# jhwang7628/openpbso

Hardware: AMD Instinct MI355X
Metric: audio samples/s & real-time x at N_obj x N_modes (higher is better)
Workload: dtype f32

## Files before the change

openpbso_amd/csrc/kernels_block.hip:

```cpp
#include <type_traits>

#include "kernels.h"
#include "wave_ops.h"

namespace pbso {
namespace iir_block {

typedef float f4 __attribute__((ext_vector_type(4)));

constexpr int BJ = BLOCK_J, BN = BLOCK_N;
constexpr int GROUP = BJ * BN;
constexpr int ST_ROW = 130;
constexpr int ST_PAIR = 260;
__host__ __device__ constexpr int park_off(int n) { return (n & 7) * ST_PAIR + (n >> 3) * 32; }
constexpr int LIT_ROW = 68;
constexpr int ST_FLOATS = BLOCK_STAGE_FLOATS;
constexpr int RING = BLOCK_RING_FLOATS;
constexpr int FTM_U_ROW = 36;
constexpr int H_ROW = 72;
constexpr int H_PLANE = BN * H_ROW;
static_assert(BN * ST_ROW <= ST_FLOATS && 8 * ST_PAIR <= BN * ST_ROW && BJ * LIT_ROW <= ST_FLOATS && 2 * H_PLANE <= ST_FLOATS, "staging area");

struct BlkDims {
    int nb, m_pad, b_pad, frames, n_groups;
// ... 79 lines not shown
    float *__restrict__ b_qn = p_qnorm + ((size_t)obj * p.qn_nb + p.qn_b0) * p.m_pad + team.col0;
    constexpr bool HALF = R == 1;
    constexpr int RINGF = HALF ? BLOCK_HALF_RING_FLOATS : RING;
    constexpr int WAVE_FLOATS = ST_FLOATS + 2 * RINGF;
    float *stage = lds + wave * WAVE_FLOATS;
    float *ring = stage + ST_FLOATS;

    f2 x2[R], c1[R], c2[R];
    float t[R];
    bool dead[R];
#pragma unroll
    for (int r = 0; r < R; ++r) {
        const unsigned k = r * rowlen + utid;
        if (chunked) {
            const float *__restrict__ xsrc = p_xs + 2 * (((size_t)obj * p.n_chunks + chunk) * p.m_pad + team.col0);
            x2[r] = reinterpret_cast<const f2 *>(xsrc)[k];
        } else {
            x2[r].x = (p_sq + ubase)[k];
            x2[r].y = (p_sd + ubase)[k];
        }
        c1[r].x = (p_pc + ubase)[k];
        c2[r].x = (p_pc + p.plane + ubase)[k];
        c1[r].y = (p_pc + 2 * p.plane + ubase)[k];
        c2[r].y = (p_pc + 3 * p.plane + ubase)[k];
        dead[r] = b_ca[k] == 0.f && b_cb[k] == 0.f;
    }
    f4 wreg4[PROJ == 0 ? R : 1][8];
    u4 wq[PROJ == 1 ? R : 1][8];
#pragma unroll
    for (int r = 0; r < R; ++r) {
        const float *__restrict__ wsrc = p_wtab + ((ubase + r * rowlen + 64 * wave) / 2) * 64;
        if constexpr (PROJ == 0) {
#pragma unroll
            for (int i = 0; i < 8; ++i)
#pragma unroll
                for (int jj = 0; jj < 4; ++jj) wreg4[r][i][jj] = wsrc[(8 * (lane >> 4) + i) * 64 + 16 * jj + (lane & 15)];
        } else {
            const unsigned *__restrict__ wu = reinterpret_cast<const unsigned *>(wsrc);
#pragma unroll
            for (int i = 0; i < 8; ++i)
                wq[r][i] = u4{wu[(4 * i + 0) * 64 + lane], wu[(4 * i + 1) * 64 + lane], wu[(4 * i + 2) * 64 + lane], wu[(4 * i + 3) * 64 + lane]};
        }
    }

    constexpr bool FT = FORCED && PROJ == 0 && !QN && R <= 2;
    constexpr bool FTM = FT && R == 1;
    constexpr int U_ROW = FTM_U_ROW;
    float fB[FTM ? 4 : 1][2][4];
    if constexpr (FTM) {
#pragma unroll
        for (int tl = 0; tl < 4; ++tl)
#pragma unroll
            for (int c = 0; c < 2; ++c)
#pragma unroll
                for (int ks = 0; ks < 4; ++ks)
                    fB[tl][c][ks] = (p_ftab + (size_t)(2 * (4 * ks + (lane >> 4)) + c) * p.plane + ubase)[64 * wave + 16 * tl + (lane & 15)];
    }
    float fq[FT && !FTM ? R : 1][BJ], fd[FT && !FTM ? R : 1][BJ];
    if constexpr (FT && !FTM) {
#pragma unroll
        for (int r = 0; r < R; ++r) {
#pragma unroll
            for (int i = 0; i < BJ; ++i) {
                fq[r][i] = (p_ftab + (size_t)(2 * i) * p.plane + ubase)[r * rowlen + utid];
                fd[r][i] = (p_ftab + (size_t)(2 * i + 1) * p.plane + ubase)[r * rowlen + utid];
            }
        }
    }

    constexpr bool TAPS_VALU = FORCED && PROJ == 0 && R == 1;
    float phi[TAPS_VALU ? 16 : 1];
    if constexpr (TAPS_VALU) {
        const double ea = (double)b_ca[utid], eb = (double)b_cb[utid];
        double vq = 1.0, vd = 1.0;
        phi[0] = 1.f;
#pragma unroll
        for (int d = 1; d < 16; ++d) {
            vd = ea * vd + eb * vq;
            vq = vq + vd;
            phi[d] = dead[0] ? 0.f : (float)vq;
        }
    }

    bool scaled = false;
    auto usable = [](float x) { return x >= 0x1p-20f && x <= 0x1p40f; };
    auto rescale = [&](const float (&from)[R], const float (&tn)[R]) {
        bool ok = true, same = true, unit = true;
#pragma unroll
        for (int r = 0; r < R; ++r) {
            ok = ok && usable(tn[r]);
            same = same && tn[r] == from[r];
            unit = unit && from[r] == 1.f;
        }
        ok = __all(ok);
        if (ok) {
            if (!__all(same)) {
#pragma unroll
                for (int r = 0; r < R; ++r) {
                    const float f = tn[r] / from[r];
                    x2[r].x = x2[r].x * f;
                    x2[r].y = x2[r].y * f;
                }
            }
        } else if (!__all(unit)) {
#pragma unroll
            for (int r = 0; r < R; ++r) {
                x2[r].x = x2[r].x / from[r];
                x2[r].y = x2[r].y / from[r];
            }
        }
        scaled = ok;
    };
    {
        const int row0 = chunked ? p_xtrow[(size_t)obj * p.n_chunks + chunk] : p_xfer_init[obj];
        float s0[R];
#pragma unroll
        for (int r = 0; r < R; ++r) {
            s0[r] = chunked ? 1.f : (p_ss + ubase)[r * rowlen + utid];
            const float tr = row0 >= 0 ? (float)(p_xfer_rows + (size_t)row0 * p.m_pad + team.col0)[r * rowlen + utid] : 1e7f;
            t[r] = dead[r] ? 1.f : tr;
        }
        rescale(s0, t);
    }

    const BufDesc *__restrict__ dsc = p_desc + (size_t)obj * p.nb;
    float *__restrict__ aout = team.part_row >= 0 ? p_audio_parts + (size_t)team.part_row * p.audio_stride
                                                  : p_audio + (size_t)obj * p.audio_stride;
    const int B = p.frames;

    const f4 *bsrc = reinterpret_cast<const f4 *>(stage + park_off(lane & 15) + (lane >> 4) * 64);
    f2 *wdst = reinterpret_cast<f2 *>(stage + (lane >> 4) * 64 + 2 * (lane & 15));
    auto park = [&](int n, f2 v) { wdst[park_off(n) / 2] = v; };
    const f4 *lsrc = reinterpret_cast<const f4 *>(stage + (lane & 15) * LIT_ROW + (lane >> 4) * 16);

    auto wave_sync = [&]() {
        __builtin_amdgcn_fence(__ATOMIC_RELEASE, "wavefront");
        __builtin_amdgcn_wave_barrier();
        __builtin_amdgcn_fence(__ATOMIC_ACQUIRE, "wavefront");
    };


    float nca[R], ncb[R], ng11[R], ng12[R], ng22[R], ngr[R];
    const float *__restrict__ g32_obj = p_g32 + (size_t)p_g32_off[obj] * p.m_pad + team.col0;
    float *gland = lds + blockDim.x / 64 * WAVE_FLOATS + wave * (3 * R * 64);
    float ntr[R];
    auto lane_off = [&]() {
        unsigned v = utid;
        asm volatile("" : "+v"(v));
        return v;
    };
    const unsigned rowlen4 = 4u * rowlen;
    auto lane_off4 = [&]() { return 4u * lane_off(); };
    auto ld_row = [](const float *base, unsigned off) { return *reinterpret_cast<const float *>(reinterpret_cast<const char *>(base) + off); };
    auto st_row = [](float *base, unsigned off, float v) { *reinterpret_cast<float *>(reinterpret_cast<char *>(base) + off) = v; };
    const int dump_row = DUMP ? p_dump_row[obj] : -1;
    int dump_b = 0;
    auto dump_state = [&](int r, int blk) {
        if (DUMP && dump_row >= 0) {
            f2 *dst = reinterpret_cast<f2 *>(p_xdump) + (((size_t)dump_row * p.qn_nb + dump_b) * 32 + blk) * p.m_pad + team.col0;
            dst[r * rowlen + lane_off()] = x2[r];
        }
    };
    auto dump_scale = [&](int code) {
        if (DUMP && dump_row >= 0) {
            float *dst = p_xscale + ((size_t)dump_row * p.qn_nb + dump_b) * p.m_pad + team.col0;
            const unsigned off = lane_off4();
#pragma unroll
            for (int r = 0; r < R; ++r) st_row(dst, off + r * rowlen4, code > 0 ? t[r] : (float)code);
        }
    };
    auto prefetch_gq = [&]() {
        if (QN) {
            const unsigned off = lane_off4();
#pragma unroll
            for (int r = 0; r < R; ++r) {
                ng11[r] = ld_row(b_gq, off + r * rowlen4);
                ng12[r] = ld_row(b_gq + p.plane, off + r * rowlen4);
                ng22[r] = ld_row(b_gq + 2 * p.plane, off + r * rowlen4);
            }
        }
    };
    auto prefetch = [&](const BufDesc &nd, bool with_gq = true) {
        const unsigned off = lane_off4();
#pragma unroll
        for (int r = 0; r < R; ++r) {
            nca[r] = ld_row(b_ca, off + r * rowlen4);
            ncb[r] = ld_row(b_cb, off + r * rowlen4);
        }
        if (with_gq) prefetch_gq();
        if (nd.frow >= 0 && !(nd.flags & DESC_DIRECT)) {
            const float *__restrict__ gsrc = p_grows + (size_t)nd.frow * p.m_pad + team.col0;
#pragma unroll
            for (int r = 0; r < R; ++r) ngr[r] = ld_row(gsrc, off + r * rowlen4);
        }
        if (nd.trow >= 0) {
            const double *__restrict__ tsrc = p_xfer_rows + (size_t)nd.trow * p.m_pad + team.col0;
#pragma unroll
            for (int r = 0; r < R; ++r)
                ntr[r] = (float)*reinterpret_cast<const double *>(reinterpret_cast<const char *>(tsrc) + 2u * (off + r * rowlen4));
        }
    };

    const unsigned gland_addr = (unsigned)(size_t)gland;
    auto prefetch_direct = [&](const BufDesc &nd) {
        if (nd.frow >= 0 && (nd.flags & DESC_DIRECT)) {
            const unsigned voff = 4u * lane_off();
#pragma unroll
            for (int k = 0; k < 3; ++k) {
#pragma unroll
                for (int r = 0; r < R; ++r) {
                    const float *__restrict__ row = g32_obj + (size_t)(nd.frow + k) * p.m_pad + r * rowlen;
                    asm volatile("s_mov_b32 m0, %0\n\tglobal_load_lds_dword %1, %2"
                                 :: "s"(gland_addr + (unsigned)((k * R + r) * 256)), "v"(voff), "s"(row) : "memory", "m0");
                }
            }
        }
    };

    const unsigned park_base = (unsigned)(size_t)wdst;
    unsigned park_row[4];
#pragma unroll
    for (int j = 0; j < 4; ++j) park_row[j] = park_base + j * 2 * ST_PAIR * 4;
    auto step_p = [&](int r) {
        float qa, da, qn, dn;
        asm volatile("v_fma_f32 %0, %1, %2, %2" : "=v"(qa) : "v"(c1[r].x), "v"(x2[r].x));
        asm volatile("v_mul_f32 %0, %1, %2" : "=v"(da) : "v"(c1[r].y), "v"(x2[r].x));
        asm volatile("v_fma_f32 %0, %1, %2, %3" : "=v"(qn) : "v"(c2[r].x), "v"(x2[r].y), "v"(qa));
        asm volatile("v_fma_f32 %0, %1, %2, %3" : "=v"(dn) : "v"(c2[r].y), "v"(x2[r].y), "v"(da));
        x2[r].x = qn;
        x2[r].y = dn;
    };
#define PBSO_PK_PAIR(J, O0, O1)                                                                   \
    "v_pk_fma_f32 %[t], %[c1], %[x], %[x] op_sel_hi:[1,0,1]\n\t"                                   \
    "v_pk_fma_f32 %[y], %[c2], %[x], %[t] op_sel:[0,1,0] op_sel_hi:[1,1,1]\n\t"                    \
    "ds_write2_b64 %[a" #J "], %[x], %[y] offset0:" #O0 " offset1:" #O1 "\n\t"                      \
    "v_pk_fma_f32 %[t], %[c1], %[y], %[y] op_sel_hi:[1,0,1]\n\t"                                   \
    "v_pk_fma_f32 %[x], %[c2], %[y], %[t] op_sel:[0,1,0] op_sel_hi:[1,1,1]\n\t"
    static_assert(ST_PAIR / 2 == 130, "offsets of the ds_write2_b64 pairs below (8-byte units): blocks n, n + 1 are rows 130 apart, n + 8 is 16 further");
    auto vburst_pk = [&](int r) {
        f2 t, y;
        const f2 c2m = f2{c2[r].x, c2[r].y - 1.f};
        asm volatile(PBSO_PK_PAIR(0, 0, 130) PBSO_PK_PAIR(1, 0, 130) PBSO_PK_PAIR(2, 0, 130) PBSO_PK_PAIR(3, 0, 130)
                     PBSO_PK_PAIR(0, 16, 146) PBSO_PK_PAIR(1, 16, 146) PBSO_PK_PAIR(2, 16, 146) PBSO_PK_PAIR(3, 16, 146)
                     : [x] "+v"(x2[r]), [t] "=&v"(t), [y] "=&v"(y)
                     : [c1] "v"(c1[r]), [c2] "v"(c2m), [a0] "v"(park_row[0]), [a1] "v"(park_row[1]), [a2] "v"(park_row[2]), [a3] "v"(park_row[3])
                     : "memory");
    };
#undef PBSO_PK_PAIR
    auto coarse2 = [&](int r, auto nc, int blk) {
        constexpr int n = decltype(nc)::value;
        static_assert((n & 1) == 0 && park_off(n + 1) - park_off(n) == ST_PAIR, "a pair of blocks = two rows of the image");
        dump_state(r, blk);
        const f2 xa = x2[r];
        step_p(r);
        dump_state(r, blk + 1);
        asm volatile("ds_write2_b64 %0, %1, %2 offset0:%3 offset1:%4"
                     :: "v"(park_row[(n & 7) / 2]), "v"(xa), "v"(x2[r]), "n"((n >> 3) * 16), "n"((n >> 3) * 16 + ST_PAIR / 2) : "memory");
        step_p(r);
    };

    unsigned long long cy_head = 0, cy_pipe = 0, cy_bar = 0, cy_comb = 0, cy_mark = 0, cy_taps = 0, cy_step = 0;
    auto lap = [&](unsigned long long &acc) {
        if (p_census) {
            const unsigned long long now = __builtin_amdgcn_s_memtime();
            acc += now - cy_mark;
            cy_mark = now;
        }
    };
    BufDesc next = dsc[b_begin];
    prefetch(next);
    prefetch_direct(next);
    if (p_census) cy_mark = __builtin_amdgcn_s_memtime();
    int prio_rank = 0;
    if (p.rotate) {
        unsigned *word = p_board + 2048 + (((__builtin_amdgcn_s_getreg((31 << 11) | 20) & 7u) << 8) | ((__builtin_amdgcn_s_getreg((31 << 11) | 4) >> 8) & 0xFFu));
        if (tid == 0) ring[0] = __builtin_bit_cast(float, atomicAdd(word, 1u));
        __syncthreads();
        prio_rank = (int)(__builtin_bit_cast(unsigned, lds[ST_FLOATS]) & 3u);
        __syncthreads();
    }
    for (int b = b_begin; b < b_end; ++b) {
        const BufDesc cur = next;
        next = dsc[b + 1 < p.nb ? b + 1 : b];
        auto set_pipe_prio = [&]() {
            if (p.rotate) {
                switch ((prio_rank + b - b_begin) & 3) {
                case 0: __builtin_amdgcn_s_setprio(0); break;
                case 1: __builtin_amdgcn_s_setprio(1); break;
                case 2: __builtin_amdgcn_s_setprio(2); break;
                default: __builtin_amdgcn_s_setprio(3); break;
                }
            }
        };
        set_pipe_prio();

        const int frow = cur.frow;
        const int prow = (cur.flags & DESC_DIRECT) ? -1 : cur.prow;
        const float amp = cur.amp;
        const int trow = cur.trow;
        const uint32_t flags = cur.flags;
        float *rg = ring + (b & 1) * RING;
        auto ring_grp = [&](int grp) { return HALF ? ring + grp * RINGF : rg + GROUP * grp; };
        auto ring_s0 = [&]() { return HALF ? ring + GROUP : rg + GROUP * NG; };
        auto combine_half = [&](int grp) {
            if constexpr (HALF) {
                lap(cy_pipe);
                __syncthreads();
                lap(cy_bar);
                if (wave == (2 * (b - b_begin) + grp) % W) {
                    const float *r0 = lds + ST_FLOATS + grp * RINGF;
                    float *__restrict__ ao = aout + (size_t)b * B + GROUP * grp;
                    const unsigned j = lane_off() & 63u;
                    f4 acc = *reinterpret_cast<const f4 *>(r0 + 4 * j);
                    for (int w = 1; w < W; ++w) acc += *reinterpret_cast<const f4 *>(r0 + w * WAVE_FLOATS + 4 * j);
                    AUDIO_STORE(&ao[4 * j + 1], acc.x);
                    AUDIO_STORE(&ao[4 * j + 2], acc.y);
                    AUDIO_STORE(&ao[4 * j + 3], acc.z);
                    AUDIO_STORE(&ao[4 * j + 4], acc.w);
                    if (grp == 0 && j == 0) {
                        float a0 = r0[GROUP];
                        for (int w = 1; w < W; ++w) a0 += r0[w * WAVE_FLOATS + GROUP];
                        AUDIO_STORE(&ao[0], a0);
                    }
                }
                lap(cy_comb);
            }
        };
        dump_b = p.qn_b0 + b;

        if (flags & DESC_SKIP) {
            dump_scale(-1);
            const unsigned off = lane_off4();
            for (unsigned o = off; o < 4u * (unsigned)B; o += rowlen4) st_row(aout + (size_t)b * B, o, 0.f);
            if (QN) {
#pragma unroll
                for (int r = 0; r < R; ++r) st_row(b_qn + (size_t)b * p.m_pad, off + r * rowlen4, 0.f);
            }
            prefetch(next);
            prefetch_direct(next);
            continue;
        }
        if (trow != XFER_KEEP) {
            float tn[R], from[R];
#pragma unroll
            for (int r = 0; r < R; ++r) {
                const float tr = trow >= 0 ? ntr[r] : 1e7f;
                tn[r] = dead[r] ? 1.f : tr;
                from[r] = scaled ? t[r] : 1.f;
            }
            rescale(from, tn);
#pragma unroll
            for (int v = 0; v < R; ++v) t[v] = tn[v];
        }
        float g_[R];
#pragma unroll
        for (int r = 0; r < R; ++r) {
            float gv = ngr[r];
            if (flags & DESC_DIRECT) {
                __builtin_amdgcn_s_waitcnt(0x0F70);
                const float *gl = gland + r * 64 + lane;
                gv = __builtin_bit_cast(float, cur.prow) * gl[0];
                gv = fmaf(__builtin_bit_cast(float, cur.tile_mask), gl[R * 64], gv);
                gv = fmaf(__builtin_bit_cast(float, cur.pad[0]), gl[2 * R * 64], gv);
            }
            g_[r] = frow >= 0 ? (scaled ? gv * t[r] : gv) : 0.f;
        }
        prefetch_direct(next);
        const bool impulse = (flags & DESC_IMPULSE) != 0;
        const bool dense = frow >= 0 && !impulse;

        dump_scale(scaled && !dense ? 1 : 0);
        const bool forced_block = FORCED && PROJ == 0 && scaled && dense;
        if (scaled && !dense) {
            const bool hit0 = frow >= 0 && ((flags & DESC_DIRECT) || (cur.tile_mask & 1u));
            float p0 = 0.f;
#pragma unroll
            for (int v = 0; v < R; ++v) {
                float a = nca[v] * x2[v].y;
                a = fmaf(ncb[v], x2[v].x, a);
                if (hit0) a = fmaf(g_[v], amp, a);
                x2[v].y = a;
                x2[v].x = x2[v].x + a;
                p0 = (v == 0) ? x2[v].x : p0 + x2[v].x;
            }
            if (QN) {
                const unsigned off = lane_off4();
#pragma unroll
                for (int v = 0; v < R; ++v) {
                    float e = ng22[v] * x2[v].y * x2[v].y;
                    e = fmaf(ng12[v] * x2[v].x, x2[v].y, e);
                    e = fmaf(ng11[v] * x2[v].x, x2[v].x, e);
                    const float nrm = __builtin_amdgcn_sqrtf(fmaxf(e, 0.f));
                    st_row(b_qn + (size_t)b * p.m_pad, off + v * rowlen4, nrm * __builtin_amdgcn_rcpf(t[v]));
                }
            }
            p0 = wave_sum(p0);
            if (lane == 0) *ring_s0() = p0;

            if constexpr (PROJ == 0) {
            f4 bq[8];
            lap(cy_head);
            wave_sync();
            if constexpr (!DUMP) vburst_pk(0);
            else static_for<0, BN / 2>([&](auto hc) { coarse2(0, std::integral_constant<int, 2 * decltype(hc)::value>{}, 2 * decltype(hc)::value); });
            wave_sync();
#pragma unroll
            for (int i = 0; i < 8; ++i) bq[i] = bsrc[i];
            f4 acc0, acc1;
            static_for<0, U>([&](auto uc) {
                constexpr int u = decltype(uc)::value;
                constexpr int r = u % R, grp = u / R;
                constexpr int rn = (u + 1) % R;
                constexpr bool more = u + 1 < U;
                if constexpr (r == 0) {
                    acc0 = f4{0.f, 0.f, 0.f, 0.f};
                    acc1 = f4{0.f, 0.f, 0.f, 0.f};
                }
                wave_sync();
                __builtin_amdgcn_sched_barrier(0);
                if constexpr (more) {
                    if constexpr (!DUMP) vburst_pk(rn);
                    else static_for<0, BN / 2>([&](auto hc) {
                        constexpr int n = 2 * decltype(hc)::value;
                        coarse2(rn, std::integral_constant<int, n>{}, BN * ((u + 1) / R) + n);
                    });
                    wave_sync();
                }
                __builtin_amdgcn_sched_barrier(0);
                static_for<0, 32>([&](auto sc) {
                    constexpr int s = decltype(sc)::value;
                    if constexpr (s & 1) acc1 = __builtin_amdgcn_mfma_f32_16x16x4f32(wreg4[r][s >> 2][s & 3], bq[s >> 2][s & 3], acc1, 0, 0, 0);
                    else acc0 = __builtin_amdgcn_mfma_f32_16x16x4f32(wreg4[r][s >> 2][s & 3], bq[s >> 2][s & 3], acc0, 0, 0, 0);
                    if constexpr (more && (s & 3) == 3 && s >= 7) bq[(s >> 2) - 1] = bsrc[(s >> 2) - 1];
                    if constexpr (!more && s == 15) prefetch(next, false);
                    __builtin_amdgcn_sched_barrier(0);
                });
                if constexpr (more) bq[7] = bsrc[7];
                else prefetch_gq();
                if constexpr (r == R - 1) {
                    const f4 acc = acc0 + acc1;
                    const unsigned l = lane_off() & 63u;
                    *reinterpret_cast<f4 *>(ring_grp(grp) + 16 * (l & 15u) + 4 * (l >> 4)) = acc;
                    combine_half(grp);
                }
            });
            } else {
                unsigned *hdst = reinterpret_cast<unsigned *>(stage) + lane;
                const u4 *hsrc = reinterpret_cast<const u4 *>(reinterpret_cast<const unsigned *>(stage) + (lane & 15) * H_ROW + 4 * (lane >> 4));
                auto coarse16 = [&](int r, int n, int blk) {
                    dump_state(r, blk);
                    const f2 x = x2[r];
                    const float xq = x.x, xd = x.y;
                    const unsigned hq = __builtin_bit_cast(unsigned, xq) & 0xFFFF0000u;
                    const unsigned hd = __builtin_bit_cast(unsigned, xd) & 0xFFFF0000u;
                    const unsigned hp = __builtin_amdgcn_perm(hd, hq, 0x07060302u);
                    const float lq = xq - __builtin_bit_cast(float, hq), ld = xd - __builtin_bit_cast(float, hd);
                    const unsigned lp = __builtin_amdgcn_perm(__builtin_bit_cast(unsigned, ld), __builtin_bit_cast(unsigned, lq), 0x07060302u);
                    hdst[n * H_ROW] = hp;
                    hdst[H_PLANE + n * H_ROW] = lp;
                    const float qa = fmaf(c1[r].x, x.x, x.x);
                    const float da = c1[r].y * x.x;
                    x2[r].x = fmaf(c2[r].x, x.y, qa);
                    x2[r].y = fmaf(c2[r].y, x.y, da);
                };
                u4 breg[8];
                lap(cy_head);
                wave_sync();
#pragma unroll
                for (int n = 0; n < BN; ++n) coarse16(0, n, n);
                wave_sync();
#pragma unroll
                for (int g = 0; g < 4; ++g) {
                    breg[2 * g] = hsrc[4 * g];
                    breg[2 * g + 1] = hsrc[H_PLANE / 4 + 4 * g];
                }
                f4 acc0, acc1;
                static_for<0, U>([&](auto uc) {
                    constexpr int u = decltype(uc)::value;
                    constexpr int r = u % R, grp = u / R;
                    constexpr int rn = (u + 1) % R;
                    constexpr bool more = u + 1 < U;
                    if constexpr (r == 0) {
                        acc0 = f4{0.f, 0.f, 0.f, 0.f};
                        acc1 = f4{0.f, 0.f, 0.f, 0.f};
                    }
                    wave_sync();
                    __builtin_amdgcn_sched_barrier(0);
                    static_for<0, BN>([&](auto nc) {
                        constexpr int n = decltype(nc)::value;
                        if constexpr (more) coarse16(rn, n, BN * ((u + 1) / R) + n);
                        if constexpr (n >= 4) {
                            constexpr int k = n - 4, g = k / 3, which = k % 3;
                            const u4 wh = wq[r][2 * g], wl = wq[r][2 * g + 1];
                            if constexpr (which == 0)
                                acc0 = __builtin_amdgcn_mfma_f32_16x16x32_bf16(__builtin_bit_cast(bf16x8, wh), __builtin_bit_cast(bf16x8, breg[2 * g]), acc0, 0, 0, 0);
                            else if constexpr (which == 1)
                                acc1 = __builtin_amdgcn_mfma_f32_16x16x32_bf16(__builtin_bit_cast(bf16x8, wh), __builtin_bit_cast(bf16x8, breg[2 * g + 1]), acc1, 0, 0, 0);
                            else
                                acc0 = __builtin_amdgcn_mfma_f32_16x16x32_bf16(__builtin_bit_cast(bf16x8, wl), __builtin_bit_cast(bf16x8, breg[2 * g]), acc0, 0, 0, 0);
                        }
                        __builtin_amdgcn_sched_barrier(0);
                    });
                    if constexpr (more) {
                        wave_sync();
#pragma unroll
                        for (int g = 0; g < 4; ++g) {
                            breg[2 * g] = hsrc[4 * g];
                            breg[2 * g + 1] = hsrc[H_PLANE / 4 + 4 * g];
                        }
                    } else {
                        prefetch(next);
                    }
                    if constexpr (r == R - 1) {
                        const f4 acc = acc0 + acc1;
                        const unsigned l = lane_off() & 63u;
                        *reinterpret_cast<f4 *>(ring_grp(grp) + 16 * (l & 15u) + 4 * (l >> 4)) = acc;
                        combine_half(grp);
                    }
                });
            }
        } else if (forced_block) {
            if constexpr (PROJ == 0 && FORCED) {
            const float *__restrict__ tprow = p_tprof + (size_t)(prow >= 0 ? prow : 0) * p.b_pad;
            float *taps = stage + BN * ST_ROW;
            float qn[R];
            lap(cy_head);
            constexpr bool FIR_EARLY = R <= 2;
            float fir_ball[FIR_EARLY ? NG : 1][4];
            if constexpr (FIR_EARLY) {
#pragma unroll
                for (int grp = 0; grp < NG; ++grp)
#pragma unroll
                    for (int kk = 0; kk < 4; ++kk) fir_ball[grp][kk] = tprow[1 + GROUP * grp + BJ * (lane & 15) + 4 * kk + (lane >> 4)];
            }
            {
                const float tk0 = tprow[0];
                float p0 = 0.f, gs = 0.f;
#pragma unroll
                for (int v = 0; v < R; ++v) {
                    float a = nca[v] * x2[v].y;
                    a = fmaf(ncb[v], x2[v].x, a);
                    a = fmaf(g_[v], tk0, a);
                    x2[v].y = a;
                    x2[v].x = x2[v].x + a;
                    p0 = (v == 0) ? x2[v].x : p0 + x2[v].x;
                    gs = (v == 0) ? g_[v] : gs + g_[v];
                    qn[v] = x2[v].x * x2[v].x;
                }
                p0 = wave_sum(p0);
                if (!TAPS_VALU) gs = wave_sum(gs);
                if (lane == 0) *ring_s0() = p0;
                wave_sync();
                if (!TAPS_VALU && lane == 0) taps[0] = gs;
            }
            f4 bq[8];
            if constexpr (TAPS_VALU) {
                float pv[16];
#pragma unroll
                for (int d = 0; d < 16; ++d) pv[d] = g_[0] * phi[d];
                const float hd = wave_sum16(pv, lane, stage + ST_ROW, wave_sync);
                if (lane < 16) taps[taps_index(lane)] = hd;
                wave_sync();
            } else {
                f4 ah0 = f4{0.f, 0.f, 0.f, 0.f}, ah1 = f4{0.f, 0.f, 0.f, 0.f};
                static_for<0, R>([&](auto rc) {
                    constexpr int r = decltype(rc)::value;
                    if constexpr (r > 0) wave_sync();
                    park(0, f2{g_[r], g_[r]});
                    wave_sync();
#pragma unroll
                    for (int i = 0; i < 8; ++i) bq[i] = bsrc[i];
                    static_for<0, 32>([&](auto sc) {
                        constexpr int s2 = decltype(sc)::value;
                        if constexpr (s2 & 1) ah1 = __builtin_amdgcn_mfma_f32_16x16x4f32(wreg4[r][s2 >> 2][s2 & 3], bq[s2 >> 2][s2 & 3], ah1, 0, 0, 0);
                        else ah0 = __builtin_amdgcn_mfma_f32_16x16x4f32(wreg4[r][s2 >> 2][s2 & 3], bq[s2 >> 2][s2 & 3], ah0, 0, 0, 0);
                    });
                });
                const f4 ah = ah0 + ah1;
                if ((lane & 15) == 0) {
                    float *td = taps + 1 + 4 * (lane >> 4);
                    td[0] = ah.x; td[1] = ah.y; td[2] = ah.z; td[3] = ah.w;
                }
                wave_sync();
            }
            lap(cy_taps);
            float fir_a[4];
#pragma unroll
            for (int kk = 0; kk < 4; ++kk) {
                const int idx = (lane & 15) - 4 * kk - (lane >> 4);
                fir_a[kk] = idx >= 0 ? taps[idx] : 0.f;
            }
            static_for<0, NG>([&](auto gc) {
                constexpr int grp = decltype(gc)::value;
                f4 acc0 = f4{0.f, 0.f, 0.f, 0.f}, acc1 = f4{0.f, 0.f, 0.f, 0.f};
                float fir_b[4];
#pragma unroll
                for (int kk = 0; kk < 4; ++kk)
                    fir_b[kk] = FIR_EARLY ? fir_ball[FIR_EARLY ? grp : 0][kk] : tprow[1 + GROUP * grp + BJ * (lane & 15) + 4 * kk + (lane >> 4)];
                static_for<0, R>([&](auto rc) {
                    constexpr int r = decltype(rc)::value;
                    wave_sync();
                    typedef float f4u __attribute__((ext_vector_type(4), aligned(4)));
                    auto for_each_block = [&](auto &&body) {
                        if constexpr (R == 1 && FT) {
// ... 64 lines not shown
                        wave_sync();
                        f4 uq[4], ud[4];
                        {
                            const f4 *src = reinterpret_cast<const f4 *>(ua + lane * U_ROW);
#pragma unroll
                            for (int i = 0; i < 4; ++i) { uq[i] = src[i]; ud[i] = src[4 + i]; }
                        }
                        static_for<0, BN>([&](auto nc) {
                            constexpr int n = decltype(nc)::value;
                            park(n, x2[r]);
                            const float qa = fmaf(c1[r].x, x2[r].x, x2[r].x);
                            const float da = c1[r].y * x2[r].x;
                            const float qn_ = fmaf(c2[r].x, x2[r].y, qa);
                            const float dn_ = fmaf(c2[r].y, x2[r].y, da);
                            x2[r].x = fmaf(gr, uq[n / 4][n % 4], qn_);
                            x2[r].y = fmaf(gr, ud[n / 4][n % 4], dn_);
                        });
                    } else if constexpr (FT) {
                        for_each_block([&](const float (&tv)[BJ], int n) {
                            park(n, x2[r]);
                            float uq0 = fq[r][0] * tv[0], uq1 = fq[r][1] * tv[1], ud0 = fd[r][0] * tv[0], ud1 = fd[r][1] * tv[1];
#pragma unroll
                            for (int i = 2; i < BJ; i += 2) {
                                uq0 = fmaf(fq[r][i], tv[i], uq0);
                                uq1 = fmaf(fq[r][i + 1], tv[i + 1], uq1);
                                ud0 = fmaf(fd[r][i], tv[i], ud0);
                                ud1 = fmaf(fd[r][i + 1], tv[i + 1], ud1);
                            }
                            const float qa = fmaf(c1[r].x, x2[r].x, x2[r].x);
                            const float da = c1[r].y * x2[r].x;
                            const float qn_ = fmaf(c2[r].x, x2[r].y, qa);
                            const float dn_ = fmaf(c2[r].y, x2[r].y, da);
                            x2[r].x = fmaf(gr, uq0 + uq1, qn_);
                            x2[r].y = fmaf(gr, ud0 + ud1, dn_);
                        });
                    } else {
                        const float gi = __builtin_amdgcn_rcpf(gr);
                        f2 z = f2{x2[r].x * gi, x2[r].y * gi};
                        const bool z_ok = gr != 0.f && fabsf(gi) < 0x1p100f && fabsf(z.x) < 0x1p50f && fabsf(z.y) < 0x1p50f;
                        if (__all(z_ok)) {
                            float qz = 0.f;
                            for_each_block([&](const float (&tv)[BJ], int n) {
                                park(n, f2{gr * z.x, gr * z.y});
#pragma unroll
                                for (int k = 0; k < BJ; ++k) {
                                    const float in = fmaf(nca[r], z.y, tv[k]);
                                    z.y = fmaf(ncb[r], z.x, in);
                                    z.x = z.x + z.y;
                                    if (QN) qz = fmaf(z.x, z.x, qz);
                                }
                            });
                            x2[r] = f2{gr * z.x, gr * z.y};
                            if (QN) qn[r] = fmaf(gr * gr, qz, qn[r]);
                        } else {
                            for_each_block([&](const float (&tv)[BJ], int n) {
                                park(n, x2[r]);
#pragma unroll
                                for (int k = 0; k < BJ; ++k) {
                                    const float gt = g_[r] * tv[k];
                                    const float in = fmaf(nca[r], x2[r].y, gt);
                                    x2[r].y = fmaf(ncb[r], x2[r].x, in);
                                    x2[r].x = x2[r].x + x2[r].y;
                                    if (QN) qn[r] = fmaf(x2[r].x, x2[r].x, qn[r]);
                                }
                            });
                        }
                    }
                    lap(cy_step);
                    wave_sync();
#pragma unroll
                    for (int i = 0; i < 8; ++i) bq[i] = bsrc[i];
                    static_for<0, 32>([&](auto sc) {
                        constexpr int s2 = decltype(sc)::value;
                        if constexpr (s2 & 1) acc1 = __builtin_amdgcn_mfma_f32_16x16x4f32(wreg4[r][s2 >> 2][s2 & 3], bq[s2 >> 2][s2 & 3], acc1, 0, 0, 0);
                        else acc0 = __builtin_amdgcn_mfma_f32_16x16x4f32(wreg4[r][s2 >> 2][s2 & 3], bq[s2 >> 2][s2 & 3], acc0, 0, 0, 0);
                    });
                });
#pragma unroll
                for (int kk = 0; kk < 4; ++kk) {
                    if (kk & 1) acc1 = __builtin_amdgcn_mfma_f32_16x16x4f32(fir_a[kk], fir_b[kk], acc1, 0, 0, 0);
                    else acc0 = __builtin_amdgcn_mfma_f32_16x16x4f32(fir_a[kk], fir_b[kk], acc0, 0, 0, 0);
                }
                const f4 acc = acc0 + acc1;
                const unsigned l = lane_off() & 63u;
                *reinterpret_cast<f4 *>(ring_grp(grp) + 16 * (l & 15u) + 4 * (l >> 4)) = acc;
                combine_half(grp);
            });
            if (QN) {
                const unsigned off = lane_off4();
#pragma unroll
                for (int r = 0; r < R; ++r) st_row(b_qn + (size_t)b * p.m_pad, off + r * rowlen4, sqrtf(qn[r]) / t[r]);
            }
            prefetch(next);
            }
        } else {
            const float *__restrict__ tprow = p_tprof + (size_t)(prow >= 0 ? prow : 0) * p.b_pad;
            float qn[R];
#pragma unroll
            for (int r = 0; r < R; ++r) qn[r] = 0.f;
            auto step1 = [&](float tk, bool forced) {
                float pp = 0.f;
#pragma unroll
                for (int v = 0; v < R; ++v) {
                    float a = nca[v] * x2[v].y;
                    a = fmaf(ncb[v], x2[v].x, a);
                    if (forced) a = fmaf(g_[v], tk, a);
                    x2[v].y = a;
                    x2[v].x = x2[v].x + a;
                    if (scaled) pp = (v == 0) ? x2[v].x : pp + x2[v].x;
                    else pp = (v == 0) ? t[v] * x2[v].x : fmaf(t[v], x2[v].x, pp);
                    if (QN) qn[v] = fmaf(x2[v].x, x2[v].x, qn[v]);
                }
                return pp;
            };
            {
                const float tk0 = dense ? tprow[0] : ((frow >= 0 && ((flags & DESC_DIRECT) || (cur.tile_mask & 1u))) ? amp : 0.f);
                float p0 = step1(tk0, frow >= 0);
                p0 = wave_sum(p0);
                if (lane == 0) *ring_s0() = p0;
            }
            for (int c = 0; c < NG * BN; ++c) {
                wave_sync();
#pragma unroll 4
                for (int k = 0; k < BJ; ++k) {
                    const float tk = dense ? tprow[1 + c * BJ + k] : 0.f;
                    const float pp = step1(tk, dense);
                    stage[k * LIT_ROW + lane] = pp;
                }
                wave_sync();
                float rs = 0.f;
#pragma unroll
                for (int j = 0; j < 4; ++j) {
                    const f4 v = lsrc[j];
                    rs += v.x;
                    rs += v.y;
                    rs += v.z;
                    rs += v.w;
                }
                rs += __shfl_xor(rs, 16, 64);
                rs += __shfl_xor(rs, 32, 64);
                if (lane < BJ) ring_grp(c / BN)[(c % BN) * BJ + lane] = rs;
                if (HALF && (c % BN) == BN - 1) combine_half(c / BN);
            }
            if (QN) {
                const unsigned off = lane_off4();
#pragma unroll
                for (int r = 0; r < R; ++r) {
                    const float nrm = sqrtf(qn[r]);
                    st_row(b_qn + (size_t)b * p.m_pad, off + r * rowlen4, scaled ? nrm / t[r] : nrm);
                }
            }
            prefetch(next);
        }

        if constexpr (!HALF) {
        lap(cy_pipe);
        __syncthreads();
        lap(cy_bar);
        {
            const float *r0 = lds + ST_FLOATS + (b & 1) * RING;
            float *__restrict__ ao = aout + (size_t)b * B;
            for (int j = (int)lane_off(); j < GROUP * NG / 4; j += blockDim.x) {
                f4 acc = *reinterpret_cast<const f4 *>(r0 + 4 * j);
                float a0 = r0[GROUP * NG];
                for (int w = 1; w < W; ++w) {
                    const f4 v = *reinterpret_cast<const f4 *>(r0 + w * WAVE_FLOATS + 4 * j);
                    const float v0 = r0[w * WAVE_FLOATS + GROUP * NG];
                    __builtin_amdgcn_sched_barrier(0);
                    acc += v;
                    a0 += v0;
                }
                float *__restrict__ aj = reinterpret_cast<float *>(reinterpret_cast<char *>(ao) + 16u * (unsigned)j);
                AUDIO_STORE(&aj[1], acc.x);
                AUDIO_STORE(&aj[2], acc.y);
                AUDIO_STORE(&aj[3], acc.z);
                AUDIO_STORE(&aj[4], acc.w);
                if (j == 0) AUDIO_STORE(&ao[0], a0);
            }
        }
        lap(cy_comb);
        }
    }

    if (p_census && tid == 0) {
        const size_t census_row = (size_t)team.id + (size_t)chunk * p.census_stride;
        p_census[census_row * CENSUS_WORDS + 0] = census_t0;
        p_census[census_row * CENSUS_WORDS + 1] = __builtin_amdgcn_s_memrealtime();
        p_census[census_row * CENSUS_WORDS + 2] = __builtin_amdgcn_s_getreg((31 << 11) | 4);
        p_census[census_row * CENSUS_WORDS + 3] = __builtin_amdgcn_s_getreg((31 << 11) | 20);
        p_census[census_row * CENSUS_WORDS + 4] = census_c0;
        p_census[census_row * CENSUS_WORDS + 5] = __builtin_amdgcn_s_memtime();
        p_census[census_row * CENSUS_WORDS + 6] = cy_head;
        p_census[census_row * CENSUS_WORDS + 7] = cy_pipe;
        p_census[census_row * CENSUS_WORDS + 8] = cy_bar;
        p_census[census_row * CENSUS_WORDS + 9] = cy_comb;
        p_census[census_row * CENSUS_WORDS + 10] = cy_taps;
        p_census[census_row * CENSUS_WORDS + 11] = cy_step;
    }
    if (chunked) return;
    const unsigned utid_end = lane_off();
#pragma unroll
    for (int r = 0; r < R; ++r) {
        const unsigned k = r * rowlen + utid_end;
        (p_sq + ubase)[k] = x2[r].x;
        (p_sd + ubase)[k] = x2[r].y;
        (p_ss + ubase)[k] = scaled ? t[r] : 1.f;
    }
}

template <int R, int QNM, int PROJ, bool DUMP, bool FORCED = false, bool CHUNKED = false>
static int launch_one(const IirParams &p, int n_teams, int W, hipStream_t stream) {
    if constexpr (!CHUNKED && !DUMP) {
        if (p.tc_cb > 0) return launch_one<R, QNM, PROJ, DUMP, FORCED, true>(p, n_teams, W, stream);
    }
    if (!CHUNKED && p.tc_cb > 0) return (int)hipErrorInvalidValue;
    const size_t lds = block_lds_bytes(W, R);
    constexpr int MAXT = 64 * MAX_WAVES_PER_BLOCK_TEAM;
    if (64 * W > MAXT) return (int)hipErrorInvalidValue;
    auto kern = iir_block_kernel<R, QNM, PROJ, DUMP, MAXT, FORCED, CHUNKED>;
    if (lds > 64 * 1024) {
        hipError_t e = hipFuncSetAttribute(reinterpret_cast<const void *>(kern),
                                           hipFuncAttributeMaxDynamicSharedMemorySize, (int)lds);
        if (e != hipSuccess) return (int)e;
    }
    const int frames = p.frames;
    const int n_chunks = p.tc_cb > 0 ? (p.nb + p.tc_cb - 1) / p.tc_cb : 1;
    const BlkDims dims = {p.nb, p.m_pad, p.b_pad, frames, (frames - 1) / GROUP, p.audio_stride, p.gq_plane, p.qn_nb, p.qn_b0, p.rotate_prio, p.forced_block,
                          p.tc_cb, n_chunks, p.census_stride, p.start_flag, p.start_seq};
    hipLaunchKernelGGL(kern, dim3(n_teams, n_chunks), dim3(64 * W), lds, stream, p.ca, p.cb, p.sq, p.sd, p.ss, p.desc, p.grows, p.g32, p.g32_off,
                       p.tprof, p.xfer_rows, p.xfer_init, p.audio, p.qnorm, p.gq, p.pc, p.wtab, p.teams, p.audio_parts, p.census, p.xdump, p.xscale, p.dump_row, p.board, p.ftab,
                       p.tc_xs, p.tc_xtrow, dims);
    return (int)hipGetLastError();
}

template <int R>
static int launch_r(const IirParams &p, int n_teams, int W, bool qn, int proj, hipStream_t s) {
    if (p.xdump) {
        return proj ? launch_one<R, 2, 1, true>(p, n_teams, W, s) : launch_one<R, 2, 0, true>(p, n_teams, W, s);
    }
    if (proj) return qn ? launch_one<R, 2, 1, false>(p, n_teams, W, s) : launch_one<R, 0, 1, false>(p, n_teams, W, s);
    if (p.forced_block) return qn ? launch_one<R, 2, 0, false, true>(p, n_teams, W, s) : launch_one<R, 0, 0, false, true>(p, n_teams, W, s);
    return qn ? launch_one<R, 2, 0, false>(p, n_teams, W, s) : launch_one<R, 0, 0, false>(p, n_teams, W, s);
}

int launch_block_r1(const IirParams &p, int n_teams, int W, bool qn, int proj, hipStream_t s);
int launch_block_r2(const IirParams &p, int n_teams, int W, bool qn, int proj, hipStream_t s);
#if !defined(PBSO_ONLY_R4) && (!defined(PBSO_BLOCK_PART) || PBSO_BLOCK_PART == 1)
int launch_block_r1(const IirParams &p, int n_teams, int W, bool qn, int proj, hipStream_t s) { return launch_r<1>(p, n_teams, W, qn, proj, s); }
int launch_block_r2(const IirParams &p, int n_teams, int W, bool qn, int proj, hipStream_t s) { return launch_r<2>(p, n_teams, W, qn, proj, s); }
#endif

#if !defined(PBSO_BLOCK_PART) || PBSO_BLOCK_PART == 0
int launch_iir_block(const IirParams &p, int n_teams, int R, int W, int qnm, int proj, hipStream_t s) {
    if (n_teams <= 0) return 0;
    if (W < 1 || W > MAX_WAVES_PER_BLOCK_TEAM) return (int)hipErrorInvalidValue;
    if (p.frames != 1 + 2 * GROUP) return (int)hipErrorInvalidValue;
    const bool qn = qnm != 0;
    switch (R) {
#ifndef PBSO_ONLY_R4
    case 1: return launch_block_r1(p, n_teams, W, qn, proj, s);
    case 2: return launch_block_r2(p, n_teams, W, qn, proj, s);
#endif
    case 4: return launch_r<4>(p, n_teams, W, qn, proj, s);
    }
// ... 79 lines not shown
```

Baseline: 52.70 billion.

## Restructure per-buffer control flow into uniform scalar branches and cache reciprocals

Turns the if/else chain over skip, block, forced and general paths into separate branches on wave-uniform scalar conditions hidden behind asm barriers. Prefetch of the next buffer's coefficients and rows now happens once at the end, or early inside the block path once the tap loop finishes. The change also caches reciprocal scales, precomputes the ring accumulator lane address, and splits the rescale logic so the divide is shared. The aim is to reduce divergence-driven exec-mask handling, register pressure and redundant address math in the hot loop. The cost is more fragile compiler-steering code and a possible change in where loads overlap.

```diff
diff --git a/openpbso_amd/csrc/kernels_block.hip b/openpbso_amd/csrc/kernels_block.hip
--- a/openpbso_amd/csrc/kernels_block.hip
+++ b/openpbso_amd/csrc/kernels_block.hip
@@ -185,8 +185,14 @@
         }
     }
 
-    bool scaled = false;
+    int scaled = 0;
     auto usable = [](float x) { return x >= 0x1p-20f && x <= 0x1p40f; };
+    auto opaque = [](int c) {
+        int v = c;
+        asm volatile("" : "+s"(v));
+        return v != 0;
+    };
+    auto into_home = [](float &home, float v) { asm volatile("v_mov_b32 %0, %1" : "+v"(home) : "v"(v)); };
     auto rescale = [&](const float (&from)[R], const float (&tn)[R]) {
         bool ok = true, same = true, unit = true;
 #pragma unroll
@@ -196,23 +202,28 @@
             unit = unit && from[r] == 1.f;
         }
         ok = __all(ok);
-        if (ok) {
-            if (!__all(same)) {
-#pragma unroll
-                for (int r = 0; r < R; ++r) {
-                    const float f = tn[r] / from[r];
-                    x2[r].x = x2[r].x * f;
-                    x2[r].y = x2[r].y * f;
-                }
-            }
-        } else if (!__all(unit)) {
+        const bool mul = ok && !__all(same), div = !ok && !__all(unit);
+        const int mul_s = __builtin_amdgcn_readfirstlane((int)mul), div_s = __builtin_amdgcn_readfirstlane((int)div);
+        float quo[R];
+        if (mul_s | div_s) {
+#pragma unroll
+            for (int r = 0; r < R; ++r) quo[r] = (mul_s ? tn[r] : x2[r].x) / from[r];
+        }
+        if (opaque(mul_s)) {
 #pragma unroll
             for (int r = 0; r < R; ++r) {
-                x2[r].x = x2[r].x / from[r];
+                x2[r].x = x2[r].x * quo[r];
+                x2[r].y = x2[r].y * quo[r];
+            }
+        }
+        if (opaque(div_s)) {
+#pragma unroll
+            for (int r = 0; r < R; ++r) {
+                x2[r].x = quo[r];
                 x2[r].y = x2[r].y / from[r];
             }
         }
-        scaled = ok;
+        scaled = __builtin_amdgcn_readfirstlane((int)ok);
     };
     {
         const int row0 = chunked ? p_xtrow[(size_t)obj * p.n_chunks + chunk] : p_xfer_init[obj];
@@ -225,7 +236,16 @@
         }
         rescale(s0, t);
     }
-
+    float rt[R];
+#pragma unroll
+    for (int r = 0; r < R; ++r) rt[r] = __builtin_amdgcn_rcpf(t[r]);
+
+    unsigned deadv[R];
+#pragma unroll
+    for (int r = 0; r < R; ++r) {
+        deadv[r] = dead[r] ? 1u : 0u;
+        asm volatile("" : "+v"(deadv[r]));
+    }
     const BufDesc *__restrict__ dsc = p_desc + (size_t)obj * p.nb;
     float *__restrict__ aout = team.part_row >= 0 ? p_audio_parts + (size_t)team.part_row * p.audio_stride
                                                   : p_audio + (size_t)obj * p.audio_stride;
@@ -235,6 +255,7 @@
     f2 *wdst = reinterpret_cast<f2 *>(stage + (lane >> 4) * 64 + 2 * (lane & 15));
     auto park = [&](int n, f2 v) { wdst[park_off(n) / 2] = v; };
     const f4 *lsrc = reinterpret_cast<const f4 *>(stage + (lane & 15) * LIT_ROW + (lane >> 4) * 16);
+    float *ring_lane = ring + 16 * (lane & 15) + 4 * (lane >> 4);
 
     auto wave_sync = [&]() {
         __builtin_amdgcn_fence(__ATOMIC_RELEASE, "wavefront");
@@ -247,13 +268,13 @@
     const float *__restrict__ g32_obj = p_g32 + (size_t)p_g32_off[obj] * p.m_pad + team.col0;
     float *gland = lds + blockDim.x / 64 * WAVE_FLOATS + wave * (3 * R * 64);
     float ntr[R];
-    auto lane_off = [&]() {
-        unsigned v = utid;
-        asm volatile("" : "+v"(v));
-        return v;
-    };
+    unsigned lane4 = 4u * utid;
+    auto lane_off4 = [&]() {
+        asm volatile("" : "+v"(lane4));
+        return lane4;
+    };
+    auto lane_off = [&]() { return lane_off4() >> 2; };
     const unsigned rowlen4 = 4u * rowlen;
-    auto lane_off4 = [&]() { return 4u * lane_off(); };
     auto ld_row = [](const float *base, unsigned off) { return *reinterpret_cast<const float *>(reinterpret_cast<const char *>(base) + off); };
     auto st_row = [](float *base, unsigned off, float v) { *reinterpret_cast<float *>(reinterpret_cast<char *>(base) + off) = v; };
     const int dump_row = DUMP ? p_dump_row[obj] : -1;
@@ -283,24 +304,36 @@
             }
         }
     };
-    auto prefetch = [&](const BufDesc &nd, bool with_gq = true) {
+    auto prefetch_rows = [&](const BufDesc &nd) {
+        const unsigned off = lane_off4();
+        if (__builtin_expect(nd.frow >= 0 && !(nd.flags & DESC_DIRECT), 0)) {
+            const float *__restrict__ gsrc = p_grows + (size_t)nd.frow * p.m_pad + team.col0;
+#pragma unroll
+            for (int r = 0; r < R; ++r) ngr[r] = ld_row(gsrc, off + r * rowlen4);
+        } else {
+#pragma unroll
+            for (int r = 0; r < R; ++r) asm volatile("" : "=v"(ngr[r]));
+        }
+        if (__builtin_expect(nd.trow >= 0, 0)) {
+            const double *__restrict__ tsrc = p_xfer_rows + (size_t)nd.trow * p.m_pad + team.col0;
+#pragma unroll
+            for (int r = 0; r < R; ++r)
+                ntr[r] = (float)*reinterpret_cast<const double *>(reinterpret_cast<const char *>(tsrc) + 2u * (off + r * rowlen4));
+        } else {
+#pragma unroll
+            for (int r = 0; r < R; ++r) asm volatile("" : "=v"(ntr[r]));
+        }
+    };
+    auto prefetch = [&](const BufDesc &nd, bool with_rest = true) {
         const unsigned off = lane_off4();
 #pragma unroll
         for (int r = 0; r < R; ++r) {
             nca[r] = ld_row(b_ca, off + r * rowlen4);
             ncb[r] = ld_row(b_cb, off + r * rowlen4);
         }
-        if (with_gq) prefetch_gq();
-        if (nd.frow >= 0 && !(nd.flags & DESC_DIRECT)) {
-            const float *__restrict__ gsrc = p_grows + (size_t)nd.frow * p.m_pad + team.col0;
-#pragma unroll
-            for (int r = 0; r < R; ++r) ngr[r] = ld_row(gsrc, off + r * rowlen4);
-        }
-        if (nd.trow >= 0) {
-            const double *__restrict__ tsrc = p_xfer_rows + (size_t)nd.trow * p.m_pad + team.col0;
-#pragma unroll
-            for (int r = 0; r < R; ++r)
-                ntr[r] = (float)*reinterpret_cast<const double *>(reinterpret_cast<const char *>(tsrc) + 2u * (off + r * rowlen4));
+        if (with_rest) {
+            prefetch_gq();
+            prefetch_rows(nd);
         }
     };
 
@@ -405,6 +438,7 @@
         float *rg = ring + (b & 1) * RING;
         auto ring_grp = [&](int grp) { return HALF ? ring + grp * RINGF : rg + GROUP * grp; };
         auto ring_s0 = [&]() { return HALF ? ring + GROUP : rg + GROUP * NG; };
+        auto ring_acc = [&](int grp) { return reinterpret_cast<f4 *>(ring_lane + (HALF ? grp * RINGF : (b & 1) * RING + GROUP * grp)); };
         auto combine_half = [&](int grp) {
             if constexpr (HALF) {
                 lap(cy_pipe);
@@ -431,7 +465,7 @@
         };
         dump_b = p.qn_b0 + b;
 
-        if (flags & DESC_SKIP) {
+        if (__builtin_expect((flags & DESC_SKIP) != 0, 0)) {
             dump_scale(-1);
             const unsigned off = lane_off4();
             for (unsigned o = off; o < 4u * (unsigned)B; o += rowlen4) st_row(aout + (size_t)b * B, o, 0.f);
@@ -439,51 +473,63 @@
 #pragma unroll
                 for (int r = 0; r < R; ++r) st_row(b_qn + (size_t)b * p.m_pad, off + r * rowlen4, 0.f);
             }
-            prefetch(next);
             prefetch_direct(next);
-            continue;
-        }
-        if (trow != XFER_KEEP) {
+        }
+        int fetched = 0;
+        if (opaque(!(flags & DESC_SKIP))) {
+        if (__builtin_expect(trow != XFER_KEEP, 0)) {
             float tn[R], from[R];
 #pragma unroll
             for (int r = 0; r < R; ++r) {
                 const float tr = trow >= 0 ? ntr[r] : 1e7f;
-                tn[r] = dead[r] ? 1.f : tr;
+                asm volatile("" : "+v"(deadv[r]));
+                tn[r] = deadv[r] != 0u ? 1.f : tr;
                 from[r] = scaled ? t[r] : 1.f;
             }
             rescale(from, tn);
 #pragma unroll
-            for (int v = 0; v < R; ++v) t[v] = tn[v];
+            for (int v = 0; v < R; ++v) {
+                into_home(t[v], tn[v]);
+                rt[v] = __builtin_amdgcn_rcpf(t[v]);
+            }
         }
         float g_[R];
 #pragma unroll
-        for (int r = 0; r < R; ++r) {
-            float gv = ngr[r];
-            if (flags & DESC_DIRECT) {
-                __builtin_amdgcn_s_waitcnt(0x0F70);
-                const float *gl = gland + r * 64 + lane;
-                gv = __builtin_bit_cast(float, cur.prow) * gl[0];
-                gv = fmaf(__builtin_bit_cast(float, cur.tile_mask), gl[R * 64], gv);
-                gv = fmaf(__builtin_bit_cast(float, cur.pad[0]), gl[2 * R * 64], gv);
-            }
-            g_[r] = frow >= 0 ? (scaled ? gv * t[r] : gv) : 0.f;
+        for (int r = 0; r < R; ++r) g_[r] = 0.f;
+        if (frow >= 0) {
+#pragma unroll
+            for (int r = 0; r < R; ++r) {
+                float gv = ngr[r];
+                if (flags & DESC_DIRECT) {
+                    __builtin_amdgcn_s_waitcnt(0x0F70);
+                    const float *gl = gland + r * 64 + lane;
+                    gv = __builtin_bit_cast(float, cur.prow) * gl[0];
+                    gv = fmaf(__builtin_bit_cast(float, cur.tile_mask), gl[R * 64], gv);
+                    gv = fmaf(__builtin_bit_cast(float, cur.pad[0]), gl[2 * R * 64], gv);
+                }
+                g_[r] = scaled ? gv * t[r] : gv;
+            }
         }
         prefetch_direct(next);
-        const bool impulse = (flags & DESC_IMPULSE) != 0;
-        const bool dense = frow >= 0 && !impulse;
+        const int impulse = (flags & DESC_IMPULSE) != 0;
+        const int dense = (int)(frow >= 0) & (impulse ^ 1);
 
         dump_scale(scaled && !dense ? 1 : 0);
-        const bool forced_block = FORCED && PROJ == 0 && scaled && dense;
-        if (scaled && !dense) {
+        const int forced_block = (FORCED && PROJ == 0) ? (scaled & dense) : 0;
+        const int block_path = scaled & (dense ^ 1);
+        if (__builtin_expect(block_path, 1)) {
             const bool hit0 = frow >= 0 && ((flags & DESC_DIRECT) || (cur.tile_mask & 1u));
-            float p0 = 0.f;
+            float p0 = 0.f, a0[R];
+#pragma unroll
+            for (int v = 0; v < R; ++v) a0[v] = fmaf(ncb[v], x2[v].x, nca[v] * x2[v].y);
+            if (hit0) {
+#pragma unroll
+                for (int v = 0; v < R; ++v) a0[v] = fmaf(g_[v], amp, a0[v]);
+            }
 #pragma unroll
             for (int v = 0; v < R; ++v) {
-                float a = nca[v] * x2[v].y;
-                a = fmaf(ncb[v], x2[v].x, a);
-                if (hit0) a = fmaf(g_[v], amp, a);
-                x2[v].y = a;
-                x2[v].x = x2[v].x + a;
+                x2[v].y = a0[v];
+                x2[v].x = x2[v].x + a0[v];
                 p0 = (v == 0) ? x2[v].x : p0 + x2[v].x;
             }
             if (QN) {
@@ -494,7 +540,7 @@
                     e = fmaf(ng12[v] * x2[v].x, x2[v].y, e);
                     e = fmaf(ng11[v] * x2[v].x, x2[v].x, e);
                     const float nrm = __builtin_amdgcn_sqrtf(fmaxf(e, 0.f));
-                    st_row(b_qn + (size_t)b * p.m_pad, off + v * rowlen4, nrm * __builtin_amdgcn_rcpf(t[v]));
+                    st_row(b_qn + (size_t)b * p.m_pad, off + v * rowlen4, nrm * rt[v]);
                 }
             }
             p0 = wave_sum(p0);
@@ -539,11 +585,14 @@
                     __builtin_amdgcn_sched_barrier(0);
                 });
                 if constexpr (more) bq[7] = bsrc[7];
-                else prefetch_gq();
+                else {
+                    prefetch_gq();
+                    prefetch_rows(next);
+                    fetched = 1;
+                }
                 if constexpr (r == R - 1) {
                     const f4 acc = acc0 + acc1;
-                    const unsigned l = lane_off() & 63u;
-                    *reinterpret_cast<f4 *>(ring_grp(grp) + 16 * (l & 15u) + 4 * (l >> 4)) = acc;
+                    *ring_acc(grp) = acc;
                     combine_half(grp);
                 }
             });
@@ -613,16 +662,17 @@
                         }
                     } else {
                         prefetch(next);
+                        fetched = 1;
                     }
                     if constexpr (r == R - 1) {
                         const f4 acc = acc0 + acc1;
-                        const unsigned l = lane_off() & 63u;
-                        *reinterpret_cast<f4 *>(ring_grp(grp) + 16 * (l & 15u) + 4 * (l >> 4)) = acc;
+                        *ring_acc(grp) = acc;
                         combine_half(grp);
                     }
                 });
             }
-        } else if (forced_block) {
+        }
+        if (opaque((block_path ^ 1) & forced_block)) {
             if constexpr (PROJ == 0 && FORCED) {
             const float *__restrict__ tprow = p_tprof + (size_t)(prow >= 0 ? prow : 0) * p.b_pad;
             float *taps = stage + BN * ST_ROW;
@@ -853,8 +903,7 @@
                     else acc0 = __builtin_amdgcn_mfma_f32_16x16x4f32(fir_a[kk], fir_b[kk], acc0, 0, 0, 0);
                 }
                 const f4 acc = acc0 + acc1;
-                const unsigned l = lane_off() & 63u;
-                *reinterpret_cast<f4 *>(ring_grp(grp) + 16 * (l & 15u) + 4 * (l >> 4)) = acc;
+                *ring_acc(grp) = acc;
                 combine_half(grp);
             });
             if (QN) {
@@ -862,9 +911,9 @@
 #pragma unroll
                 for (int r = 0; r < R; ++r) st_row(b_qn + (size_t)b * p.m_pad, off + r * rowlen4, sqrtf(qn[r]) / t[r]);
             }
-            prefetch(next);
-            }
-        } else {
+            }
+        }
+        if (opaque((block_path ^ 1) & (forced_block ^ 1))) {
             const float *__restrict__ tprow = p_tprof + (size_t)(prow >= 0 ? prow : 0) * p.b_pad;
             float qn[R];
 #pragma unroll
@@ -921,7 +970,6 @@
                     st_row(b_qn + (size_t)b * p.m_pad, off + r * rowlen4, scaled ? nrm / t[r] : nrm);
                 }
             }
-            prefetch(next);
         }
 
         if constexpr (!HALF) {
@@ -951,6 +999,8 @@
         }
         lap(cy_comb);
         }
+        }
+        if (opaque(fetched ^ 1)) prefetch(next);
     }
 
     if (p_census && tid == 0) {
```

Result: no change. 52.80 billion (median of 6 runs) (+0.2%).
